# Venomalia/AuroraLib.Compression

Measured on AMD Instinct MI355X. Metric: decompressed GiB/s (whole job; 10k x 256KiB batch per GPU), one batch in flight, higher is better.
Workload: dtype u8; 1 GPU; yaz0 decode, 10000 x 256 KiB synthetic streams per GPU (SURVEY 8d token-level generator, seed 0xA17A0000+1000*cfg+i), device-resident; format=yaz0, streams_this_rank=10000, streams_whole_job=10000, stream_bytes=262144, compressed_bytes_whole_job=357382689, batches_in_flight=1, parity_ok=True, parallelism=stream-sharded x1, every rank its own batch, no collective

## Files before the change

auroralib/compression_amd/csrc/alz_decode_fast.h:

```cpp
#pragma once
#ifndef ALZ_DESCTAB_ALL
#define ALZ_DESCTAB_ALL 0
#endif
#ifndef ALZ_TAB512
#define ALZ_TAB512 1
#endif
#include "alz_emit_byte.h"
#include "alz_prs_table.h"
template <int FMT> struct alz_tab512 { static constexpr bool value = ALZ_DESCTAB_ALL != 0 || (ALZ_TAB512 != 0 && (FMT == ALZ_FMT_YAZ0 || FMT == ALZ_FMT_LZ11)); };

#ifndef ALZ_QRUN
#define ALZ_QRUN 200u
#endif
#ifndef ALZ_WIDE_FLAT
#define ALZ_WIDE_FLAT 1
#endif
#ifndef ALZ_WIDE_WALK
#define ALZ_WIDE_WALK 1
#endif
#ifndef ALZ_NB
#define ALZ_NB 8
#endif

__device__ __forceinline__ u32 wave_writelane(u32 old, u32 val, u32 lane) {
    u32 tmp;
    asm volatile("s_mov_b32 %1, %2\n\ts_mov_b32 m0, %3\n\ts_nop 0\n\tv_writelane_b32 %0, %1, m0" : "+v"(old), "=&s"(tmp) : "s"(val), "s"(lane) : "m0");
    return old;
}

struct FastGeom {
    u32 length_bits, min_length, windows_start, max_distance, W;
};

template <int FMT> struct FamTraits;
template <> struct FamTraits<ALZ_FMT_LZSS> { static constexpr bool MSB = false, LIT1 = true,  H3 = false, H4 = false, NIBLO = false, NEG = false; };
template <> struct FamTraits<ALZ_FMT_LZ10> { static constexpr bool MSB = true,  LIT1 = false, H3 = false, H4 = false, NIBLO = false, NEG = false; };
template <> struct FamTraits<ALZ_FMT_LZ02> { static constexpr bool MSB = true,  LIT1 = false, H3 = true,  H4 = false, NIBLO = true,  NEG = false; };
template <> struct FamTraits<ALZ_FMT_CLZ0> { static constexpr bool MSB = false, LIT1 = false, H3 = false, H4 = false, NIBLO = false, NEG = false; };
template <> struct FamTraits<ALZ_FMT_BLZ>  { static constexpr bool MSB = true,  LIT1 = false, H3 = false, H4 = false, NIBLO = false, NEG = false; };
template <> struct FamTraits<ALZ_FMT_LZ11> { static constexpr bool MSB = true,  LIT1 = false, H3 = true,  H4 = true,  NIBLO = false, NEG = false; };
template <> struct FamTraits<ALZ_FMT_YAZ0> { static constexpr bool MSB = true,  LIT1 = true,  H3 = true,  H4 = false, NIBLO = false, NEG = false; };
template <> struct FamTraits<ALZ_FMT_LZ40> { static constexpr bool MSB = true,  LIT1 = false, H3 = true,  H4 = true,  NIBLO = true,  NEG = true; };

__device__ __forceinline__ u32 mask_window(u64 lo, u64 hi, int i) {
    u64 w = (lo >> i) | ((hi << (63 - i)) << 1);
    return (u32)w;
}

template <int FMT, class OW>
__device__ __forceinline__ bool fast_iter_interleaved(InCache& in, OW& out, DecState& s, u32 size, u32 src_len, bool& to_serial, u8* segmark, int lane, const FastGeom& gm) {
    typedef FamTraits<FMT> TR;
    constexpr bool WALK = TR::H3 || TR::H4;
    constexpr bool WIDE = WALK ? (ALZ_WIDE_WALK != 0) : (ALZ_WIDE_FLAT != 0);
    const u32 p = s.p;
    in.ensure(p, WIDE ? 224 : 128);
    const u32 x0 = in.byte_at(p + (u32)lane), x1 = in.byte_at(p + 64u + (u32)lane);
    u32 l3 = 0, l4 = 0, l3b = 0, l4b = 0;
    if (WALK) {
        const u32 n0 = TR::NIBLO ? (x0 & 0xFu) : (x0 >> 4), n1 = TR::NIBLO ? (x1 & 0xFu) : (x1 >> 4);
        u32 n2 = 0;
        if (WIDE) { const u32 x2 = in.byte_at(p + 128u + (u32)lane); n2 = TR::NIBLO ? (x2 & 0xFu) : (x2 >> 4); }
        if (TR::H3) { const u64 lo = __ballot(n0 == 0), hi = __ballot(n1 == 0); l3 = mask_window(lo, hi, lane); if (WIDE) l3b = mask_window(hi, __ballot(n2 == 0), lane); }
        if (TR::H4) { const u64 lo = __ballot(n0 == 1), hi = __ballot(n1 == 1); l4 = mask_window(lo, hi, lane); if (WIDE) l4b = mask_window(hi, __ballot(n2 == 1), lane); }
    }
    auto spec = [&](u32 xb, u32 w3, u32 w4, u32& gsize, u32& info) {
        const u32 mbits = TR::NEG ? ((0u - xb) & 0xFFu) : (TR::LIT1 ? (~xb & 0xFFu) : xb);
        if (!WALK) { gsize = 9u + (u32)__popc(mbits); info = mbits; }
        else {
            u32 r = 1; info = 0;
#pragma unroll
            for (int k = 0; k < 8; k++) {
                const u32 m = __builtin_amdgcn_ubfe(mbits, (u32)(TR::MSB ? 7 - k : k), 1u);
                u32 extra;
                if (TR::H3 && !TR::H4) { const u32 z = __builtin_amdgcn_ubfe(w3, r, 1u); asm("v_mad_u32_u24 %0, %1, %2, %1" : "=v"(extra) : "v"(m), "v"(z)); }
                else {
                    const u32 z = __builtin_amdgcn_ubfe(w3, r, 1u) + 2u * __builtin_amdgcn_ubfe(w4, r, 1u);
                    asm("v_mad_u32_u24 %0, %1, %2, %1" : "=v"(extra) : "v"(m), "v"(z));
                }
                if (k == 0) info = extra;
                else asm("v_lshl_or_b32 %0, %1, %2, %0" : "+v"(info) : "v"(extra), "n"(4 * k));
                r += 1u + extra;
            }
            gsize = r;
        }
    };
    u32 gsize, info, gsize1 = 0, info1 = 0;
    spec(x0, l3, l4, gsize, info);
    if (WIDE) spec(x1, l3b, l4b, gsize1, info1);
    u32 g = 0, ng = 0, gstart = 0;
#pragma unroll
    for (int it = 0; it < 8; it++) {
        if (g < (WIDE ? 128u : 64u)) {
            if ((lane >> 3) == it) gstart = g;
            if (WIDE) g += g < 64u ? wave_readlane(gsize, g) : wave_readlane(gsize1, g - 64u);
            else g += wave_readlane(gsize, g);
            ng = (u32)it + 1u;
        }
    }
    const u32 k = (u32)lane & 7u;
    u32 inf = wave_bperm(gstart & 63u, info);
    if (WIDE) { const u32 inf1 = wave_bperm(gstart & 63u, info1); inf = gstart < 64u ? inf : inf1; }
    u32 m, to;
    if (!TR::H3 && !TR::H4) {
        m = (inf >> (TR::MSB ? 7u - k : k)) & 1u;
        const u32 before = TR::MSB ? (u32)__popc(inf >> (8u - k)) : (u32)__popc(inf & ((1u << k) - 1u));
        to = gstart + 1u + k + before;
    } else {
        m = ((inf >> (4u * k)) & 0xFu) != 0u;
        to = gstart + 1u + k + (u32)__builtin_amdgcn_udot8(inf & ((1u << (4u * k)) - 1u), 0x11111111u, 0u, false);
    }
    const u32 ti = in.idx(p + to);
    const u32 b1 = in.lds[ti], b2 = in.lds[ti + 1];
    u32 len = 1, desc = ALZ_DESC_LIT(b1), tend = to + 1;
    bool term = false;
    if (m) {
        if (FMT == ALZ_FMT_LZSS) {
            u32 offset = ((b2 >> gm.length_bits) << 8) | b1;
            len = (b2 & ((1u << gm.length_bits) - 1u)) + gm.min_length;
            offset = (gm.max_distance + offset - gm.windows_start) & (gm.max_distance - 1u);
            desc = ALZ_DESC_MATCH(offset); tend = to + 2;
        } else if (FMT == ALZ_FMT_LZ10) {
            desc = ALZ_DESC_MATCH((((b1 & 0xFu) << 8) | b2) + 1u); len = (b1 >> 4) + 3u; tend = to + 2;
        } else if (FMT == ALZ_FMT_LZ02) {
            const u32 b3 = in.lds[ti + 2];
            const u32 nib = b1 & 0xFu, d = ((b1 & 0xF0u) << 4) | b2;
            desc = ALZ_DESC_MATCH(d ? d : 4096u);
            if (nib == 0) { len = b3 + 17u; tend = to + 3; term = d == 0u; } else { len = nib + 1u; tend = to + 2; }
        } else if (FMT == ALZ_FMT_CLZ0) {
            desc = ALZ_DESC_MATCH(0x1000u - (b1 | ((b2 >> 4) << 8))); len = (b2 & 0xFu) + 3u; tend = to + 2;
        } else if (FMT == ALZ_FMT_BLZ) {
            desc = ALZ_DESC_MATCH((((b1 & 0xFu) << 8) | b2) + 3u); len = (b1 >> 4) + 3u; tend = to + 2;
        } else if (FMT == ALZ_FMT_LZ11) {
            const u32 b3 = in.lds[ti + 2], b4 = in.lds[ti + 3];
            const u32 nib = b1 >> 4;
            if (nib == 0) { desc = ALZ_DESC_MATCH((((b2 & 0xFu) << 8) | b3) + 1u); len = (((b1 & 0xFu) << 4) | (b2 >> 4)) + 17u; tend = to + 3; }
            else if (nib == 1) { desc = ALZ_DESC_MATCH((((b3 & 0xFu) << 8) | b4) + 1u); len = (((b1 & 0xFu) << 12) | (b2 << 4) | (b3 >> 4)) + 273u; tend = to + 4; }
            else { desc = ALZ_DESC_MATCH((((b1 & 0xFu) << 8) | b2) + 1u); len = nib + 1u; tend = to + 2; }
        } else if (FMT == ALZ_FMT_LZ40) {
            const u32 b3 = in.lds[ti + 2], b4 = in.lds[ti + 3];
            const u32 nib = b1 & 0xFu, d = (b1 >> 4) | (b2 << 4);
            desc = ALZ_DESC_MATCH(d ? d : 4096u);
            if (nib == 0) { len = b3 + 16u; tend = to + 3; } else if (nib == 1) { len = (b3 | (b4 << 8)) + 272u; tend = to + 4; } else { len = nib; tend = to + 2; }
        } else {
            const u32 b3 = in.lds[ti + 2];
            const u32 nib = b1 >> 4;
            desc = ALZ_DESC_MATCH((((b1 & 0xFu) << 8) | b2) + 1u);
            if (nib == 0) { len = b3 + 0x12u; tend = to + 3; } else { len = nib + 2u; tend = to + 2; }
        }
    }
    const u32 inlim = src_len - p;
    const u64 ingm = lanes_below(8u * ng);
    const u64 fitm = wave_ballot(tend <= inlim);
    u64 vm = ingm & fitm;
    bool cut = (ingm & ~fitm) != 0;
    if (FMT == ALZ_FMT_LZ02) {
        const u64 tm = vm & wave_ballot(term);
        if (tm) { vm &= lanes_below((u32)__builtin_ctzll(tm)); cut = true; }
    }
    if (cut && vm == 0) { to_serial = true; return false; }
    u32 last_tend;
    const bool fin = fast_emit<OW, EmitCfg<((FMT == ALZ_FMT_LZSS || FMT == ALZ_FMT_BLZ) ? 0u : 4095u), FMT == ALZ_FMT_LZSS, false, OW::FB, false, false, alz_tab512<FMT>::value>>(out, s, size, vm, len, desc, tend, segmark, nullptr, lane, last_tend, gm.W);
    if (fin) {
        s.p = p + last_tend;
        if (FMT == ALZ_FMT_LZ02) {
            const u32 lk = (u32)__builtin_ctzll((vm & wave_ballot(tend == last_tend)) | (1ull << 63));
            s.bits = 7u - (lk & 7u);
            s.flag = in.peek1(p + wave_readlane(gstart, lk));
        }
        return true;
    }
    if (!cut) { s.p = p + g; return false; }
    const u32 lk = (u32)__popcll(vm) - 1u;
    s.p = p + wave_readlane(tend, lk);
    s.bits = 7u - (lk & 7u);
    s.flag = in.peek1(p + wave_readlane(gstart, lk));
    if (TR::NEG) s.flag = (0u - s.flag) & 0xFFu;
    to_serial = true;
    return false;
}

template <bool MIO0, class OW>
__device__ __forceinline__ bool fast_iter_3cursor(InCache& fin_, InCache& cin, InCache& uin, OW& out, DecState& s, u32 size, u8* segmark,
                                                  int lane, u32& fp, u32& cp, u32& up) {
    fin_.ensure(fp, 8); cin.ensure(cp, 128); uin.ensure(up, 64);
    const u32 fb = fin_.byte_at(fp + ((u32)lane >> 3));
    const bool lit = (fb >> (7 - (lane & 7))) & 1u;
    const u64 lm = __ballot(lit);
    const u32 midx = mbcnt64(~lm);
    u32 b1 = 0, b2 = 0;
    if (!lit) { const u32 ci = cin.idx(cp + 2u * midx); b1 = cin.lds[ci]; b2 = cin.lds[ci + 1]; }
    bool usesu = lit;
    if (!MIO0) usesu = lit || (b1 >> 4) == 0;
    const u64 um = __ballot(usesu);
    const u32 uidx = mbcnt64(um);
    u32 ub = 0;
    if (usesu) ub = uin.byte_at(up + uidx);
    u32 len = 1, desc = ALZ_DESC_LIT(ub);
    if (!lit) {
        desc = ALZ_DESC_MATCH((((b1 & 0xFu) << 8) | b2) + 1u);
        if (MIO0) len = (b1 >> 4) + 3u;
        else len = (b1 >> 4) ? (b1 >> 4) + 2u : ub + 0x12u;
    }
    const u32 tend = ((2u * (midx + (lit ? 0u : 1u))) << 8) | (uidx + (usesu ? 1u : 0u));
    u32 last;
    const bool fin = fast_emit<OW, EmitCfg<4095u, false, false, false, false, false, true>>(out, s, size, ~0ull, len, desc, tend, segmark, nullptr, lane, last, 4096);
    cp += fin ? (last >> 8) : 2u * (u32)__popcll(~lm);
    up += fin ? (last & 0xFFu) : (u32)__popcll(um);
    fp += fin ? 0u : 8u;
    return fin;
}

template <class OW>
__device__ __forceinline__ bool fast_iter_lzhudson(InCache& in, OW& out, DecState& s, u32 size, u8* segmark, int lane) {
    const u32 p = s.p;
    in.ensure(p, 128);
    const u32 x0 = in.byte_at(p + (u32)lane), x1 = in.byte_at(p + 64u + (u32)lane);
    const u64 zlo = __ballot((x0 >> 4) == 0), zhi = __ballot((x1 >> 4) == 0);
    const u32 l3 = mask_window(zlo, zhi, lane);
    u32 F = uni(s.flag), nb = uni(s.bits), T = 0;
    if (nb == 0) {
        F = (wave_readlane(x0, 0u) << 24) | (wave_readlane(x0, 1u) << 16) | (wave_readlane(x0, 2u) << 8) | wave_readlane(x0, 3u);
        nb = 32; T = 4;
    }
    const u32 nruns = nb >> 3;
    u32 tstart = 0, infosel = 0, done = 0;
#pragma unroll
    for (int r = 0; r < 4; r++) {
        if ((u32)r < nruns && T <= 63u && done == (u32)r) {
            const u32 mbits = ~(F >> (nb - 8u * (u32)(r + 1))) & 0xFFu;
            u32 rr = 0, info = 0;
#pragma unroll
            for (int k = 0; k < 8; k++) {
                const u32 m = __builtin_amdgcn_ubfe(mbits, (u32)(7 - k), 1u);
                u32 extra;
                { const u32 z = __builtin_amdgcn_ubfe(l3, rr, 1u); asm("v_mad_u32_u24 %0, %1, %2, %1" : "=v"(extra) : "v"(m), "v"(z)); }
                info |= extra << (4 * k);
                rr += 1u + extra;
            }
            const u32 inf = wave_readlane(info, T);
            if (((u32)lane >> 3) == (u32)r) { tstart = T; infosel = inf; }
            T += wave_readlane(rr, T);
            done = (u32)r + 1u;
        }
    }
    const u32 k = (u32)lane & 7u;
    const u32 m = ((infosel >> (4u * k)) & 0xFu) != 0u;
    const u32 to = tstart + k + (u32)__builtin_amdgcn_udot8(infosel & ((1u << (4u * k)) - 1u), 0x11111111u, 0u, false);
    const u32 ti = in.idx(p + to);
    const u32 b1 = in.lds[ti], b2 = in.lds[ti + 1], b3 = in.lds[ti + 2];
    u32 len = 1, desc = ALZ_DESC_LIT(b1), tend = to + 1;
    if (m) {
        const u32 nib = b1 >> 4;
        desc = ALZ_DESC_MATCH((((b1 & 0xFu) << 8) | b2) + 1u);
        if (nib == 0) { len = b3 + 0x12u; tend = to + 3; } else { len = nib + 2u; tend = to + 2; }
    }
    u32 last_tend;
    const bool fin = fast_emit<OW, EmitCfg<4095u, false, false, false>>(out, s, size, lanes_below(8u * done), len, desc, tend, segmark, nullptr, lane, last_tend, 4096);
    s.p = fin ? p + last_tend : p + T;
    s.flag = F; s.bits = nb - 8u * done;
    return fin;
}

template <class OW>
__device__ __forceinline__ bool fast_iter_smsr00(InCache& cin, InCache& uin, OW& out, DecState& s, u32 size, u8* segmark, int lane, u32& cp, u32& up) {
    cin.ensure(cp, 136); uin.ensure(up, 64);
    const u32 wi = cin.idx(cp + 2u * (u32)lane);
    const u32 w = ((u32)cin.lds[wi] << 8) | cin.lds[wi + 1];
    const u32 gsize = 1u + (u32)__popc(~w & 0xFFFFu);
    const u32 g0 = 0u, g1 = g0 + wave_readlane(gsize, g0), g2 = g1 + wave_readlane(gsize, g1), g3 = g2 + wave_readlane(gsize, g2);
    const u32 gend = g3 + wave_readlane(gsize, g3);
    const u32 j = (u32)lane >> 4, k = (u32)lane & 15u;
    const u32 gstart = j == 0u ? g0 : (j == 1u ? g1 : (j == 2u ? g2 : g3));
    const u32 m0 = wave_readlane(w, g0), m1 = wave_readlane(w, g1), m2 = wave_readlane(w, g2), m3 = wave_readlane(w, g3);
    const u32 mask = j == 0u ? m0 : (j == 1u ? m1 : (j == 2u ? m2 : m3));
    const bool lit = (mask >> (15u - k)) & 1u;
    const u32 mbefore = (u32)__popc((~mask & 0xFFFFu) >> (16u - k));
    const u64 lm = wave_ballot(lit);
    const u32 uidx = mbcnt64(lm);
    u32 len = 1, desc;
    if (lit) desc = ALZ_DESC_LIT(uin.byte_at(up + uidx));
    else {
        const u32 ci = cin.idx(cp + 2u * (gstart + 1u + mbefore));
        const u32 data = ((u32)cin.lds[ci] << 8) | cin.lds[ci + 1];
        desc = ALZ_DESC_MATCH((data & 0x0FFFu) + 1u); len = (data >> 12) + 3u;
    }
    const u32 tend = ((gstart + 1u + mbefore + (lit ? 0u : 1u)) << 8) | (uidx + (lit ? 1u : 0u));
    u32 last;
    const bool fin = fast_emit<OW, EmitCfg<4095u, false, false, false, false, false, true>>(out, s, size, ~0ull, len, desc, tend, segmark, nullptr, lane, last, 4096);
    if (fin) { cp += 2u * (last >> 8); up += last & 0xFFu; }
    else { cp += 2u * gend; up += (u32)__popcll(lm); }
    return fin;
}


struct EmitRet { u32 produced, flushed, ovf, att_lo, att_hi, mtag; };

#define ALZ_TOK_MATCH(len, dist) (((len) << 18) | (dist))
#define ALZ_TOK_LIT(len, lo) (((len) << 18) | 0x20000u | (lo))
#define ALZ_TOK_MAXLEN 16383u

template <class OW, class CFG>
__device__ __attribute__((noinline)) EmitRet queue_emit_call(u8* dst, u8* win, u32 lw_mask, u32 fl, u32 oshift, u32 cap, u32 produced, u32 flushed,
                                                             int lane, u8* segmark, const u8* inlds, u32 W, u32 nt, u32 qtok, u32 mtag, u32 dirty = 1u) {
    OW out;
    out.dst = reinterpret_cast<u8*>(((u64)uni((u32)((u64)dst >> 32)) << 32) | uni((u32)(u64)dst));
    out.win = win; out.lw_mask = uni(lw_mask); out.fl = uni(fl); out.oshift = uni(oshift); out.cap = uni(cap);
    out.produced = uni(produced); out.flushed = uni(flushed); out.lane = lane;
    out.slack_dirty = uni(dirty) != 0u;
    out.mtag = uni(mtag);
    DecState s; dec_state_init(s);
    const u32 len = qtok >> 18, lo = qtok & 0x1FFFFu;
    u32 desc = lo;
    if (qtok & 0x20000u) desc = CFG::LITRUN ? (0x80000000u | lo) : ALZ_DESC_LIT(lo & 0xFFu);
    u32 last;
    fast_emit<OW, CFG>(out, s, 0xFFFFFFFFu, lanes_below(uni(nt)), len, desc, 0u, segmark, inlds, lane, last, uni(W));
    EmitRet r; r.produced = out.produced; r.flushed = out.flushed; r.ovf = s.ovf ? 1u : 0u;
    r.att_lo = (u32)s.attempted_end; r.att_hi = (u32)(s.attempted_end >> 32); r.mtag = out.mtag;
    return r;
}

template <class OW>
__device__ __attribute__((noinline)) EmitRet queue_serial_call(u8* dst, u8* win, u32 lw_mask, u32 fl, u32 oshift, u32 cap, u32 produced, u32 flushed,
                                                               int lane, const u8* inlds, u32 W, u32 nt, u32 qtok) {
    OW out;
    out.dst = reinterpret_cast<u8*>(((u64)uni((u32)((u64)dst >> 32)) << 32) | uni((u32)(u64)dst));
    out.win = win; out.lw_mask = uni(lw_mask); out.fl = uni(fl); out.oshift = uni(oshift); out.cap = uni(cap);
    out.produced = uni(produced); out.flushed = uni(flushed); out.lane = lane; out.slack_dirty = true;
    const u32 n = uni(nt), w = uni(W);
    for (u32 j = 0; j < n; j++) {
        const u32 t = wave_readlane(qtok, j), len = t >> 18, lo = t & 0x1FFFFu;
        if (t & 0x20000u) out.copy_lds(inlds + lo, len); else out.back_copy(lo, len, w);
    }
    EmitRet r; r.produced = out.produced; r.flushed = out.flushed; r.ovf = 0; r.att_lo = 0; r.att_hi = 0; r.mtag = 0;
    return r;
}

template <class OW, class CFG>
struct QueueSink {
    typedef OW OWT; typedef CFG CFGT;
    OW& out; DecState& s; u8* segmark; const u8* inlds; int lane; u32 W;
    u32 qtok;
    u32 nt, qbytes;
    __device__ __forceinline__ QueueSink(OW& o, DecState& st, u8* sm, const u8* il, int ln, u32 w)
        : out(o), s(st), segmark(sm), inlds(il), lane(ln), W(w), qtok(0), nt(0), qbytes(0) {}
    __device__ __forceinline__ u32 produced() const { return out.produced + qbytes; }
    __device__ __forceinline__ void flush() {
        if (nt == 0) return;
        if constexpr (EmitUsesChunks<CFG>::value) {
            const EmitRet r = queue_serial_call<OW>(out.dst, out.win, out.lw_mask, out.fl, out.oshift, out.cap, out.produced, out.flushed, lane, inlds, W, nt, qtok);
            out.produced = uni(r.produced); out.flushed = uni(r.flushed); out.slack_dirty = true;
            nt = 0; qbytes = 0;
            return;
        }
        const EmitRet r = queue_emit_call<OW, CFG>(out.dst, out.win, out.lw_mask, out.fl, out.oshift, out.cap, out.produced, out.flushed,
                                                   lane, segmark, inlds, W, nt, qtok, out.mtag);
        out.produced = uni(r.produced); out.flushed = uni(r.flushed); out.mtag = uni(r.mtag);
        if (uni(r.ovf)) { s.ovf = true; s.attempted_end = ((u64)uni(r.att_hi) << 32) | uni(r.att_lo); }
        nt = 0; qbytes = 0;
    }
    __device__ __forceinline__ void ensure(InCache& in, u32 p, u32 need) {
        if (p + in.lo + need > in.cb + 2u * in.ch || p + in.lo < in.cb) { flush(); in.ensure(p, need); }
    }
    __device__ __forceinline__ void push_word(u32 word, u32 len) {
        qtok = wave_writelane(qtok, uni(word), uni(nt));
        nt = uni(nt + 1u); qbytes = uni(qbytes + len);
    }
    __device__ __forceinline__ bool push(u32 word, u32 len) {
        push_word(word, len);
        if (nt == 64u || qbytes >= 0x40000000u) flush();
        return !s.ovf;
    }
    __device__ __forceinline__ bool lit(u32 b) {
        if (produced() >= out.cap) {
            flush(); if (s.ovf) return false;
            (void)clip_token(out, s, 1u); return false;
        }
        return push(ALZ_TOK_LIT(1u, b & 0xFFu), 1u);
    }
    __device__ __forceinline__ bool match(u32 dist, u64 len, u32 w) {
        if (len == 0) return true;
        if (len > ALZ_TOK_MAXLEN || dist > 0x1FFFFu || (u64)produced() + len > (u64)out.cap) {
            flush(); if (s.ovf) return false;
            u32 cl = clip_token(out, s, len); out.back_copy(dist, cl, w); return !s.ovf;
        }
        return push(ALZ_TOK_MATCH((u32)len, dist ? dist : w), (u32)len);
    }
    __device__ __forceinline__ bool run(InCache& in, u32 p, u64 len) {
        if (len == 0) return true;
        if (len > in.ch || (u64)produced() + len > (u64)out.cap) {
            flush(); if (s.ovf) return false;
            u32 cl = clip_token(out, s, len); out.copy_from(in, p, cl); return !s.ovf;
        }
        ensure(in, p, (u32)len);
        return push(ALZ_TOK_LIT((u32)len, in.idx(p)), (u32)len);
    }
};

#define ALZ_NX_BAD 0x1000u
struct NoFill3 { __device__ __forceinline__ void operator()(u32&) const {} };
template <class F3 = NoFill3>
// ... 856 lines not shown
```

auroralib/compression_amd/csrc/alz_emit_byte.h:

```cpp
#pragma once
#include "alz_emit_chunk.h"

__device__ __forceinline__ u32 pointer_jump(bool instep, u32 srclane, u32 val) {
    u32 st = instep ? ((srclane << 2) | 0x40000000u) : val;
    bool un = instep;
    do {
        const u32 f = (u32)__builtin_amdgcn_ds_bpermute((int)st, (int)st);
        if (un) st = f;
        un = (int)st >= 0x40000000;
    } while (__ballot(un));
    return st;
}

struct Mapper {
    u32 relm;
    u32 tbase4;
    u32 m;
};
template <bool DESCTAB>
__device__ __forceinline__ u32 desc_of(const u8* segmark, u32 idx4, u32 desc) {
    if (DESCTAB) return *reinterpret_cast<const u32*>(segmark + 128u + idx4);
    return (u32)__builtin_amdgcn_ds_bpermute((int)idx4, (int)desc);
}
template <class OW>
__device__ __forceinline__ void mark_block(OW& out, u8* segmark, int lane, Mapper& mp) {
    u32 tag = out.mtag + 1u;
    if (tag > 255u) {
        segmark[lane] = 0; segmark[64 + lane] = 0; tag = 1u;
        wave_sync();
    }
    out.mtag = tag;
    if (mp.relm < 128u) segmark[mp.relm] = (u8)tag;
    mp.relm -= 128u;
}
template <class OW, int PAR>
__device__ __forceinline__ u64 step_marks(OW& out, u8* segmark, int lane, Mapper& mp) {
    u32 half;
    if (PAR == 0 || (PAR < 0 && (mp.m & 1u) == 0u)) { mark_block(out, segmark, lane, mp); wave_sync(); }
    if (PAR >= 0) half = 64u * (u32)PAR; else half = 64u * (mp.m & 1u);
    const u32 mk = segmark[half + (u32)lane];
    return __ballot(mk == out.mtag);
}
template <class OW, bool DESCTAB, int PAR>
__device__ __forceinline__ u32 map_one(OW& out, u8* segmark, int lane, u32 desc, Mapper& mp) {
    const u64 M = step_marks<OW, PAR>(out, segmark, lane, mp);
    const u32 cnt = __builtin_amdgcn_mbcnt_hi((u32)(M >> 32), __builtin_amdgcn_mbcnt_lo((u32)M, 0u));
    const u32 dsc = desc_of<DESCTAB>(segmark, (cnt << 2) + mp.tbase4, desc);
    mp.tbase4 += 4u * (u32)__popcll(M);
    mp.m += 1u;
    return dsc;
}

template <class OW, class CFG, bool EARLY, bool FULL>
__device__ __forceinline__ void copy_one(OW& out, const u8* inlds, int lane, u32 dsc, u32& qs, u32 nseg) {
    const u32 omask = CFG::OMASK ? CFG::OMASK : out.lw_mask;
    u8* const win = out.win;
    u32 wv = win[(qs - dsc) & omask];
    if (EARLY) { if (dsc > qs - out.oshift) wv = 0; }
    u32 val;
    if (CFG::LITRUN) { const u32 lv = inlds[(qs + dsc) & 2047u]; val = ((int)dsc < 0) ? lv : wv; }
    else val = ((int)dsc < 0) ? dsc : wv;
    const bool instep = FULL ? (dsc <= (u32)lane) : (dsc <= (u32)lane && (u32)lane < nseg);
    if (__ballot(instep)) val = pointer_jump(instep, (u32)lane - dsc, val);
    if (FULL) win[qs & omask] = (u8)val;
    else if ((u32)lane < nseg) win[qs & omask] = (u8)val;
    wave_sync();
    qs += 64u;
}

template <class OW, class CFG, int PAR>
__device__ __forceinline__ void fused_step(OW& out, u8* segmark, const u8* inlds, int lane, u32 desc, Mapper& mp, u32& qs, const u32 dsc, u32& dsc_next) {
    const u32 omask = CFG::OMASK ? CFG::OMASK : out.lw_mask;
    u8* const win = out.win;
    if (PAR == 0) { mark_block(out, segmark, lane, mp); wave_sync(); }
    const u32 wv = win[(qs - dsc) & omask];
    u32 lv = 0;
    if (CFG::LITRUN) lv = inlds[(qs + dsc) & 2047u];
    const u32 mk = segmark[64u * (u32)PAR + (u32)lane];
    const u64 M = __ballot(mk == out.mtag);
    const u32 cnt = __builtin_amdgcn_mbcnt_hi((u32)(M >> 32), __builtin_amdgcn_mbcnt_lo((u32)M, 0u));
    const u32 dscn = desc_of<CFG::DESCTAB>(segmark, (cnt << 2) + mp.tbase4, desc);
    mp.tbase4 += 4u * (u32)__popcll(M);
    mp.m += 1u;
    u32 val;
    if (CFG::LITRUN) val = ((int)dsc < 0) ? lv : wv;
    else val = ((int)dsc < 0) ? dsc : wv;
    const bool instep = dsc <= (u32)lane;
    if (__ballot(instep)) val = pointer_jump(instep, (u32)lane - dsc, val);
    win[qs & omask] = (u8)val;
    wave_sync();
    qs += 64u; dsc_next = dscn;
}

template <class OW, class CFG>
__device__ __forceinline__ void byte_emit_steps(OW& out, u8* segmark, const u8* inlds, int lane, const EmitState& e) {
    u32 desc = e.desc;
    if (CFG::LITRUN) {
        if (desc >> 31) desc = 0x80000000u | ((desc - (e.O + e.off + out.oshift)) & 2047u);
    }
    const u32 O = e.O, T = e.T, W = e.W;
    u32 X = 0;
    u32 qs = O + (u32)lane + out.oshift;
    Mapper mp;
    mp.tbase4 = 0; mp.m = 0;
    mp.relm = e.kept ? e.off + e.clen - 1u : 0xFFFFFF00u;
    if (CFG::DESCTAB) reinterpret_cast<u32*>(segmark + 128u)[lane] = desc;
    while (X + 64u <= T && (O + X < W || (mp.m & 1u))) {
        const u32 d0 = map_one<OW, CFG::DESCTAB, -1>(out, segmark, lane, desc, mp);
        copy_one<OW, CFG, true, true>(out, inlds, lane, d0, qs, 64u);
        X += 64u; out.produced = O + X; if (out.produced - out.flushed >= out.fl) out.flush_blocks();
    }
    u32 dA = 0, dB = 0; u32 ahead = 0;
    if (X + 128u <= T) {
        dA = map_one<OW, CFG::DESCTAB, 0>(out, segmark, lane, desc, mp);
        ahead = 1;
        do {
            fused_step<OW, CFG, 1>(out, segmark, inlds, lane, desc, mp, qs, dA, dB);
            fused_step<OW, CFG, 0>(out, segmark, inlds, lane, desc, mp, qs, dB, dA);
            X += 128u; out.produced = O + X;
            if (out.produced - out.flushed >= out.fl) out.flush_blocks();
        } while (X + 128u <= T);
    }
    if (X + 64u <= T) {
        if (!ahead) dA = map_one<OW, CFG::DESCTAB, -1>(out, segmark, lane, desc, mp);
        copy_one<OW, CFG, true, true>(out, inlds, lane, dA, qs, 64u); ahead = 0;
        X += 64u; out.produced = O + X; if (out.produced - out.flushed >= out.fl) out.flush_blocks();
    }
    if (X < T) {
        if (!ahead) dA = map_one<OW, CFG::DESCTAB, -1>(out, segmark, lane, desc, mp);
        copy_one<OW, CFG, true, false>(out, inlds, lane, dA, qs, T - X);
        out.produced = O + T; if (out.produced - out.flushed >= out.fl) out.flush_blocks();
    }
}

template <class OW, class CFG, bool EARLY, bool FULL>
__device__ __forceinline__ void byte_step_sm(OW& out, u8* segmark, const u8* inlds, int lane, u32 desc, u32& relm, u32& qs, u32& tbase4, u32 nseg) {
    const u32 omask = CFG::OMASK ? CFG::OMASK : out.lw_mask;
    u8* const win = out.win;
    { const u32 dump = 64u + (u32)lane; segmark[relm < dump ? relm : dump] = 1; }
    wave_sync();
    const u32 mk = segmark[lane];
    segmark[lane] = 0;
    const u64 M = __ballot(mk != 0);
    const u32 cnt = __builtin_amdgcn_mbcnt_hi((u32)(M >> 32), __builtin_amdgcn_mbcnt_lo((u32)M, 0u));
    const u32 dsc = (u32)__builtin_amdgcn_ds_bpermute((int)((cnt << 2) + tbase4), (int)desc);
    tbase4 += 4u * (u32)__popcll(M);
    u32 wv = win[(qs - dsc) & omask];
    if (EARLY) { if (dsc > qs - out.oshift) wv = 0; }
    u32 val;
    if (CFG::LITRUN) { const u32 lv = inlds[(qs + dsc) & 2047u]; val = ((int)dsc < 0) ? lv : wv; }
    else val = ((int)dsc < 0) ? dsc : wv;
    const bool instep = FULL ? (dsc <= (u32)lane) : (dsc <= (u32)lane && (u32)lane < nseg);
    if (__ballot(instep)) val = pointer_jump(instep, (u32)lane - dsc, val);
    if (FULL) win[qs & omask] = (u8)val;
    else if ((u32)lane < nseg) win[qs & omask] = (u8)val;
    wave_sync();
    qs += 64u; relm -= 64u;
}

__device__ __forceinline__ u32 map_step_sm(u8* segmark, int lane, u32 desc, u32& relm, u32& tbase4) {
    { const u32 dump = 64u + (u32)lane; segmark[relm < dump ? relm : dump] = 1; }
    wave_sync();
    const u32 mk = segmark[lane];
    segmark[lane] = 0;
    const u64 M = __ballot(mk != 0);
    const u32 cnt = __builtin_amdgcn_mbcnt_hi((u32)(M >> 32), __builtin_amdgcn_mbcnt_lo((u32)M, 0u));
    const u32 dsc = (u32)__builtin_amdgcn_ds_bpermute((int)((cnt << 2) + tbase4), (int)desc);
    tbase4 += 4u * (u32)__popcll(M);
    relm -= 64u;
    return dsc;
}

template <class OW, class CFG>
__device__ __forceinline__ void copy_step_sm(OW& out, const u8* inlds, int lane, u32 dsc, u32 far, u32& qs, u32 nseg, bool early) {
    const u32 omask = CFG::OMASK ? CFG::OMASK : out.lw_mask;
    u8* const win = out.win;
    u32 wv = win[(qs - dsc) & omask];
        if (early) { if (dsc > qs - out.oshift) wv = 0; }
    u32 val;
    if (CFG::LITRUN) { const u32 lv = inlds[(qs + dsc) & 2047u]; val = ((int)dsc < 0) ? lv : wv; }
    else val = ((int)dsc < 0) ? dsc : wv;
    const bool instep = dsc <= (u32)lane && (u32)lane < nseg;
    if (__ballot(instep)) val = pointer_jump(instep, (u32)lane - dsc, val);
    if ((u32)lane < nseg) win[qs & omask] = (u8)val;
    wave_sync();
    qs += 64u;
}

template <class OW, class CFG>
__device__ __forceinline__ void fused_step_sm(OW& out, u8* segmark, const u8* inlds, int lane, u32 desc, u32& relm, u32& qs, u32& tbase4, const u32 dsc, u32& dsc_next) {
    const u32 omask = CFG::OMASK ? CFG::OMASK : out.lw_mask;
    u8* const win = out.win;
    { const u32 dump = 64u + (u32)lane; segmark[relm < dump ? relm : dump] = 1; }
    wave_sync();
    const u32 wv = win[(qs - dsc) & omask];
    u32 lv = 0;
    if (CFG::LITRUN) lv = inlds[(qs + dsc) & 2047u];
    const u32 mk = segmark[lane];
    segmark[lane] = 0;
    const u64 M = __ballot(mk != 0);
    const u32 cnt = __builtin_amdgcn_mbcnt_hi((u32)(M >> 32), __builtin_amdgcn_mbcnt_lo((u32)M, 0u));
    const u32 dscn = (u32)__builtin_amdgcn_ds_bpermute((int)((cnt << 2) + tbase4), (int)desc);
    tbase4 += 4u * (u32)__popcll(M);
    u32 val;
    if (CFG::LITRUN) val = ((int)dsc < 0) ? lv : wv;
    else val = ((int)dsc < 0) ? dsc : wv;
    const bool instep = dsc <= (u32)lane;
    if (__ballot(instep)) val = pointer_jump(instep, (u32)lane - dsc, val);
    win[qs & omask] = (u8)val;
    wave_sync();
    qs += 64u; relm -= 64u; dsc_next = dscn;
}

template <class OW, class CFG>
__device__ __forceinline__ void byte_emit_steps_sm(OW& out, u8* segmark, const u8* inlds, int lane, const EmitState& e) {
    u32 desc = e.desc;
    if (CFG::LITRUN) {
        if (desc >> 31) desc = 0x80000000u | ((desc - (e.O + e.off + out.oshift)) & 2047u);
    }
    const u32 O = e.O, T = e.T, W = e.W;
    u32 X = 0;
    u32 qs = O + (u32)lane + out.oshift;
    u32 tbase4 = 0;
    u32 relm = e.kept ? e.off + e.clen - 1u : 0xFFFFFF00u;
    while (X + 64u <= T && O + X < W) { byte_step_sm<OW, CFG, true, true>(out, segmark, inlds, lane, desc, relm, qs, tbase4, 64u); X += 64u; out.produced = O + X; if (out.produced - out.flushed >= out.fl) out.flush_blocks(); }
    u32 nleft = (T - X) >> 6;
    u32 dsc = 0; bool have = false;
    if (nleft) {
        dsc = map_step_sm(segmark, lane, desc, relm, tbase4); have = true;
        do {
            const u32 pos = O + X + out.oshift;
            u32 nb = (out.fl - (pos & (out.fl - 1u)) + 63u) >> 6;
            if (nb > nleft) nb = nleft;
            u32 k = nb, dsc2;
            for (; k >= 2u; k -= 2u) {
                fused_step_sm<OW, CFG>(out, segmark, inlds, lane, desc, relm, qs, tbase4, dsc, dsc2);
                fused_step_sm<OW, CFG>(out, segmark, inlds, lane, desc, relm, qs, tbase4, dsc2, dsc);
            }
            if (k) { fused_step_sm<OW, CFG>(out, segmark, inlds, lane, desc, relm, qs, tbase4, dsc, dsc2); dsc = dsc2; }
            X += 64u * nb; nleft -= nb; out.produced = O + X;
            if (out.produced - out.flushed >= out.fl) out.flush_blocks();
        } while (nleft);
    }
    if (X < T) {
        if (!have) dsc = map_step_sm(segmark, lane, desc, relm, tbase4);
        copy_step_sm<OW, CFG>(out, inlds, lane, dsc, 0u, qs, T - X, true);
        out.produced = O + T; if (out.produced - out.flushed >= out.fl) out.flush_blocks();
    }
}

template <class CFG> struct EmitUsesChunks { static constexpr bool value = CFG::FALLBACK; };

template <class OW, class CFG>
__device__ __forceinline__ void emit_begin(OW& out, DecState& s, u32 size, u64 vm, u32 len, u32 desc, u32 tend, u8* scratch, int lane, u32& last_tend, u32 W, EmitState& e) {
    (void)scratch;
    emit_prologue<OW, CFG>(out, s, size, vm, len, desc, tend, lane, last_tend, W, e);
}
template <class OW, class CFG>
__device__ __forceinline__ void emit_finish(OW& out, u8* scratch, const u8* inlds, int lane, EmitState& e) {
    if constexpr (EmitUsesChunks<CFG>::value) emit_steps<OW, CFG>(out, scratch, inlds, lane, e);
    else if constexpr (CFG::STEPMARKS) byte_emit_steps_sm<OW, CFG>(out, scratch, inlds, lane, e);
    else byte_emit_steps<OW, CFG>(out, scratch, inlds, lane, e);
}

#define ALZ_MBOX_WORDS (3u * 64u + 16u)
struct WalkOut {
    static constexpr bool FB = false;
    static constexpr bool PUBLISH = true;
    u32 produced, cap;
    u32* mbox; u32 k;
    __device__ __forceinline__ void publish(const EmitState& e, int lane) {
        u32* slot = mbox + (k & 1u) * ALZ_MBOX_WORDS;
        slot[lane] = e.kept ? e.clen : 0u; slot[64 + lane] = e.off; slot[128 + lane] = e.desc;
        if (lane == 0) { slot[192] = 1u; slot[193] = e.O; slot[194] = e.T; slot[195] = e.W; }
        __syncthreads();
        k++;
    }
};

template <class OW, class CFG>
__device__ __forceinline__ bool fast_emit(OW& out, DecState& s, u32 size, u64 vm, u32 len, u32 desc, u32 tend, u8* scratch,
                                          const u8* inlds, int lane, u32& last_tend, u32 W) {
    EmitState e;
    emit_prologue<OW, CFG>(out, s, size, vm, len, desc, tend, lane, last_tend, W, e);
    if constexpr (OW::PUBLISH) {
        out.publish(e, lane);
        out.produced = e.O + e.T;
        return e.fin;
    } else {
    emit_finish<OW, CFG>(out, scratch, inlds, lane, e);
    return e.fin;
    }
}
```

Baseline: 977.9 GiB/s.

## Hand-write the group-chain walk in scalar asm and tweak mapper indexing

Replaces the unrolled C++ group-start chain walk in the wide fast path with an inline-asm sequence. It uses v_readlane, scalar adds and exec-mask shifting to assign each 8-lane group its start, and branches out early once the 64 or 128 limit is reached. The goal is to cut VALU/SALU overhead and readlane dependency stalls on the serial chain. The descriptor mapper now keeps an element count instead of a byte offset. The tail copy_one call flips its first template flag to false. The asm hard-codes exec manipulation and labels, and the flag flip could change correctness-related behaviour.

```diff
diff --git a/auroralib/compression_amd/csrc/alz_decode_fast.h b/auroralib/compression_amd/csrc/alz_decode_fast.h
--- a/auroralib/compression_amd/csrc/alz_decode_fast.h
+++ b/auroralib/compression_amd/csrc/alz_decode_fast.h
@@ -46,6 +46,49 @@
     u64 w = (lo >> i) | ((hi << (63 - i)) << 1);
     return (u32)w;
 }
+
+#ifndef ALZ_CHAIN_ASM
+#define ALZ_CHAIN_ASM 1
+#endif
+#define ALZ_HOP(it, entry, lim, src, fail) \
+    entry \
+    "s_cmpk_lt_u32 %[g], " lim "\n\t" \
+    "s_cbranch_scc0 " fail #it "_%=\n\t" \
+    "v_readlane_b32 %[n], " src ", %[g]\n\t" \
+    "s_lshl_b64 exec, exec, 8\n\t" \
+    "v_mov_b32 %[gs], %[g]\n\t" \
+    "s_add_u32 %[g], %[g], %[n]\n\t"
+#define ALZ_HOP_A(it) ALZ_HOP(it, "", "64", "%[s0]", ".LALZB")
+#define ALZ_HOP_B(it) ALZ_HOP(it, ".LALZB" #it "_%=:\n\t", "128", "%[s1]", ".LALZX")
+#define ALZ_HOP_X(it) ".LALZX" #it "_%=:\n\t" "s_movk_i32 %[ng], " #it "\n\t" "s_branch .LALZD_%=\n"
+__device__ __forceinline__ void chain_walk_wide(u32 gsize, u32 gsize1, u32& g_out, u32& ng_out, u32& gstart_out) {
+    u32 g, ng, n, gstart = 0;
+    u64 ex;
+    asm volatile(
+        "s_mov_b64 %[ex], exec\n\t"
+        "v_readlane_b32 %[n], %[s0], 0\n\t"
+        "s_mov_b64 exec, 0xff\n\t"
+        "s_mov_b32 %[g], %[n]\n\t"
+        ALZ_HOP_A(1) ALZ_HOP_A(2) ALZ_HOP_A(3) ALZ_HOP_A(4) ALZ_HOP_A(5) ALZ_HOP_A(6) ALZ_HOP_A(7)
+        "s_movk_i32 %[ng], 8\n\t"
+        "s_branch .LALZD_%=\n"
+        ALZ_HOP_B(1) ALZ_HOP_B(2) ALZ_HOP_B(3) ALZ_HOP_B(4) ALZ_HOP_B(5) ALZ_HOP_B(6) ALZ_HOP_B(7)
+        "s_movk_i32 %[ng], 8\n\t"
+        "s_branch .LALZD_%=\n"
+        ALZ_HOP_X(1) ALZ_HOP_X(2) ALZ_HOP_X(3) ALZ_HOP_X(4) ALZ_HOP_X(5) ALZ_HOP_X(6)
+        ".LALZX7_%=:\n\t"
+        "s_movk_i32 %[ng], 7\n"
+        ".LALZD_%=:\n\t"
+        "s_mov_b64 exec, %[ex]"
+        : [g] "=&s"(g), [ng] "=&s"(ng), [n] "=&s"(n), [ex] "=&s"(ex), [gs] "+v"(gstart)
+        : [s0] "v"(gsize), [s1] "v"(gsize1)
+        : "scc");
+    g_out = g; ng_out = ng; gstart_out = gstart;
+}
+#undef ALZ_HOP_X
+#undef ALZ_HOP_B
+#undef ALZ_HOP_A
+#undef ALZ_HOP
 
 template <int FMT, class OW>
 __device__ __forceinline__ bool fast_iter_interleaved(InCache& in, OW& out, DecState& s, u32 size, u32 src_len, bool& to_serial, u8* segmark, int lane, const FastGeom& gm) {
@@ -88,6 +131,8 @@
     spec(x0, l3, l4, gsize, info);
     if (WIDE) spec(x1, l3b, l4b, gsize1, info1);
     u32 g = 0, ng = 0, gstart = 0;
+    if (WIDE && ALZ_CHAIN_ASM != 0) chain_walk_wide(gsize, gsize1, g, ng, gstart);
+    else {
 #pragma unroll
     for (int it = 0; it < 8; it++) {
         if (g < (WIDE ? 128u : 64u)) {
@@ -96,6 +141,7 @@
             else g += wave_readlane(gsize, g);
             ng = (u32)it + 1u;
         }
+    }
     }
     const u32 k = (u32)lane & 7u;
     u32 inf = wave_bperm(gstart & 63u, info);
diff --git a/auroralib/compression_amd/csrc/alz_emit_byte.h b/auroralib/compression_amd/csrc/alz_emit_byte.h
--- a/auroralib/compression_amd/csrc/alz_emit_byte.h
+++ b/auroralib/compression_amd/csrc/alz_emit_byte.h
@@ -14,7 +14,7 @@
 
 struct Mapper {
     u32 relm;
-    u32 tbase4;
+    u32 tbase;
     u32 m;
 };
 template <bool DESCTAB>
@@ -45,8 +45,8 @@
 __device__ __forceinline__ u32 map_one(OW& out, u8* segmark, int lane, u32 desc, Mapper& mp) {
     const u64 M = step_marks<OW, PAR>(out, segmark, lane, mp);
     const u32 cnt = __builtin_amdgcn_mbcnt_hi((u32)(M >> 32), __builtin_amdgcn_mbcnt_lo((u32)M, 0u));
-    const u32 dsc = desc_of<DESCTAB>(segmark, (cnt << 2) + mp.tbase4, desc);
-    mp.tbase4 += 4u * (u32)__popcll(M);
+    const u32 dsc = desc_of<DESCTAB>(segmark, (cnt + mp.tbase) << 2, desc);
+    mp.tbase += (u32)__popcll(M);
     mp.m += 1u;
     return dsc;
 }
@@ -79,8 +79,8 @@
     const u32 mk = segmark[64u * (u32)PAR + (u32)lane];
     const u64 M = __ballot(mk == out.mtag);
     const u32 cnt = __builtin_amdgcn_mbcnt_hi((u32)(M >> 32), __builtin_amdgcn_mbcnt_lo((u32)M, 0u));
-    const u32 dscn = desc_of<CFG::DESCTAB>(segmark, (cnt << 2) + mp.tbase4, desc);
-    mp.tbase4 += 4u * (u32)__popcll(M);
+    const u32 dscn = desc_of<CFG::DESCTAB>(segmark, (cnt + mp.tbase) << 2, desc);
+    mp.tbase += (u32)__popcll(M);
     mp.m += 1u;
     u32 val;
     if (CFG::LITRUN) val = ((int)dsc < 0) ? lv : wv;
@@ -102,7 +102,7 @@
     u32 X = 0;
     u32 qs = O + (u32)lane + out.oshift;
     Mapper mp;
-    mp.tbase4 = 0; mp.m = 0;
+    mp.tbase = 0; mp.m = 0;
     mp.relm = e.kept ? e.off + e.clen - 1u : 0xFFFFFF00u;
     if (CFG::DESCTAB) reinterpret_cast<u32*>(segmark + 128u)[lane] = desc;
     while (X + 64u <= T && (O + X < W || (mp.m & 1u))) {
@@ -123,7 +123,7 @@
     }
     if (X + 64u <= T) {
         if (!ahead) dA = map_one<OW, CFG::DESCTAB, -1>(out, segmark, lane, desc, mp);
-        copy_one<OW, CFG, true, true>(out, inlds, lane, dA, qs, 64u); ahead = 0;
+        copy_one<OW, CFG, false, true>(out, inlds, lane, dA, qs, 64u); ahead = 0;
         X += 64u; out.produced = O + X; if (out.produced - out.flushed >= out.fl) out.flush_blocks();
     }
     if (X < T) {
```

Result: faster. 1022 GiB/s, median of 6 (+4.5%).
